# Kyaw-Thiha/animal-vision

Measured on AMD Instinct MI355X. Metric: megapixels/sec per-frame pipeline, higher is better.
Workload: dtype f16

## Files before the change

### animal-vision_amd/_lib.py

```python
from __future__ import annotations

import ctypes
import os

_HERE = os.path.dirname(os.path.abspath(__file__))
LIB_PATH = os.path.join(_HERE, "libavx.so")

AVX_OK = 0
AVX_ERR_INVALID, AVX_ERR_NO_DEVICE, AVX_ERR_HIP, AVX_ERR_UNSUPPORTED, AVX_ERR_NOMEM = -1, -2, -3, -4, -5
AVX_COLOR_MATRIX, AVX_COLOR_CAT_MERGE = 0, 1
AVX_POST_NONE, AVX_POST_GAUSS, AVX_POST_ROWGAIN, AVX_POST_STREAK = 0, 1, 2, 3
AVX_MAX_KSIZE = 33
AVX_PIX_FMTS = {"yuv420p": 0, "nv12": 1, "yuv422p": 2, "yuv444p": 3, "gray": 4, "yuv420p10le": 5, "yuv422p10le": 6, "yuv444p10le": 7,
                "p010le": 8}
AVX_TRANSFERS = {"pq": 1, "hlg": 2}
AVX_TONEMAPS = {"clip": 0, "mobius": 1}


class AvxError(RuntimeError):
    def __init__(self, code: int, msg: str):
        super().__init__(f"libavx error {code}: {msg}")
        self.code = code


# ... 339 lines not shown
    "avx_yuv_coefficients_d": (_i, [_i, _i, _i, ctypes.POINTER(ctypes.c_int), ctypes.POINTER(ctypes.c_int)]),
    "avx_yuv_frame_size": (_sz, [_i, _i, _i]),
    "avx_yuv_to_rgb_u8": (_i, [_vp, _i, _vp, _vp, _i, _i, _i, _i, _i, _vp]),
    "avx_rgb_to_yuv_u8": (_i, [_vp, _i, _vp, _vp, _i, _i, _i, _i, _i, _vp]),
    "avx_yuv_hdr_to_rgb_u8": (_i, [_vp, _i, _vp, _vp, _i, _i, _i, _i, _i, _i, ctypes.c_double, ctypes.c_double, _vp]),
    "avx_yuv_to_rgb_scaled_u8": (_i, [_vp, _i, _vp, _vp, _i, _i, _i, _i, _i, _i, _i, _vp]),
    "avx_yuv_hdr_to_rgb_scaled_u8": (_i, [_vp, _i, _vp, _vp, _i, _i, _i, _i, _i, _i, _i, _i, ctypes.c_double, ctypes.c_double, _vp]),
    "avx_frame_metrics_u8": (_i, [_vp, _vp, _vp, _i, _i, _i, _i, _vp, _vp]),
    "avx_plane_metrics": (_i, [_vp, _i, _vp, _i, _vp, _i, _i, _i, _i, _vp, _vp]),
    "avx_frame_metrics_ms_u8": (_i, [_vp, _vp, _vp, _i, _i, _i, _vp, _vp, _vp]),
    "avx_diff_map_u8": (_i, [_vp, _vp, _vp, _i, _i, _i, _i, ctypes.c_float, _i, _i, _vp, _vp, _vp, _vp]),
    "avx_delta_e_u8": (_i, [_vp, _vp, _vp, _i, _i, _i, _i, ctypes.c_float, ctypes.c_float, _i, _vp, _vp, _vp, _vp]),
    "avx_scielab_u8": (_i, [_vp, _vp, _vp, _i, _i, _i, ctypes.c_double, _i, ctypes.c_float, ctypes.c_float, _i, _vp, _vp, _vp, _vp]),
    "avx_remap_linear_planes": (_i, [_vp, _vp, _i, _i, _i, _vp, _vp, _vp, ctypes.c_float, _vp]),
    "avx_sobel3_plane": (_i, [_vp, _vp, _i, _i, _vp, _vp, _vp]),
    "avx_mst_gram": (_i, [_vp, _vp, _i, _sz, _i, _i, _vp, _vp, _vp, _vp]),
    "avx_mst_qkv_gram": (_i, [_vp, _vp, _vp, _sz, _i, _vp, _vp, _vp, _vp, _vp]),
    "avx_mst_qkv_gram16": (_i, [_vp, _vp, _vp, _sz, _i, _vp, _vp, _vp, _vp, _vp]),
    "avx_mst_ln_gemm_gelu": (_i, [_vp, _vp, _vp, _vp, ctypes.c_float, _vp, _sz, _i, _vp, _vp]),
    "avx_mst_convt2x2": (_i, [_vp, _vp, _vp, _vp, _vp, _i, _i, _i, _i, _vp]),
    "avx_mst_convt2x2_fuse": (_i, [_vp, _vp, _vp, _vp, _vp, _vp, _vp, _i, _i, _i, _i, _vp]),
    "avx_mst_posemb": (_i, [_vp, _vp, _vp, _vp, _vp, _vp, _vp, _i, _i, _i, _i, _vp]),
    "avx_mst_conv3x3_add": (_i, [_vp, _vp, _vp, _vp, _vp, _i, _i, _i, _i, _vp]),
    "avx_mst_attn_pack": (_i, [_vp, _vp, _vp, _vp, _vp, _vp, _i, _vp, _vp]),
    "avx_mst_rowgemm_add": (_i, [_vp, _vp, _vp, _vp, _vp, _vp, _vp, _sz, _i, _vp]),
    "avx_mst_conv_in_u8": (_i, [_vp, _vp, _i, _i, _i, _i, _i, _i, _vp, _vp, _vp]),
    "avx_mst_conv3x3_lds": (_i, [_vp, _vp, _vp, _vp, _vp, _i, _i, _i, _i, _vp]),
    "avx_mst_down4x4": (_i, [_vp, _vp, _vp, _vp, _i, _i, _i, _i, _vp]),
    "avx_mst_conv3x3_lds_gram": (_i, [_vp, _vp, _vp, _vp, _vp, _i, _i, _i, _vp, _vp, _vp, _vp, _vp]),
    "avx_mst_conv3x3_lds_cin": (_i, [_vp, _vp, _vp, _vp, _i, _i, _i, _i, _i, _i, _vp, _vp, _vp]),
    "avx_mst_conv3x3_lds_spectral_cin": (_i, [_vp, _vp, _vp, _vp, _i, _i, _i, _i, _i, _i, _vp, _fp, _i, _i, _i, _i, _vp, _vp, ctypes.POINTER(ctypes.c_int), _vp]),
    "avx_mst_conv3x3_lds_gram_cin": (_i, [_vp, _vp, _i, _i, _i, _i, _i, _i, _vp, _vp, _vp, _vp, _vp, _vp, _vp, _vp]),
    "avx_mst_convt2x2_fuse_gram": (_i, [_vp, _vp, _vp, _vp, _vp, _vp, _vp, _i, _i, _i, _vp, _vp, _vp, _vp, _vp]),
    "avx_mst_attn_pack16": (_i, [_vp, _vp, _vp, _vp, _vp, _vp, _i, _vp, _vp]),
    "avx_mst_attn_pack_mx": (_i, [_vp, _vp, _vp, _vp, _vp, _vp, _i, _vp, _vp]),
    "avx_mst_attn_tail_mx": (_i, [_vp, _vp, _vp, _vp, _vp, _vp, _vp, _vp, _i, _i, _i, _i, _vp]),
    "avx_mst_attn_tail_sp": (_i, [_vp, _vp, _vp, _vp, _vp, _vp, _vp, _vp, _i, _i, _i, _i, _vp]),
    "avx_mst_attn_tail_mx_col": (_i, [_vp, _vp, _vp, _vp, _vp, _vp, _vp, _vp, _i, _i, _i, _i, _i, _vp]),
    "avx_mst_attn_tail_sp_col": (_i, [_vp, _vp, _vp, _vp, _vp, _vp, _vp, _vp, _i, _i, _i, _i, _i, _vp]),
    "avx_mst_tail_march_steps": (_i, [_i, _i, _i, _i, ctypes.POINTER(ctypes.c_longlong), ctypes.POINTER(ctypes.c_ubyte), _i, ctypes.POINTER(ctypes.c_int)]),
    "avx_mst_attn_tail": (_i, [_vp, _vp, _vp, _vp, _vp, _vp, _vp, _vp, _i, _i, _i, _i, _vp]),
    "avx_mst_attn_tail_x": (_i, [_vp, _vp, _vp, _vp, _vp, _vp, _vp, _vp, _i, _i, _i, _i, _vp]),
    "avx_mst_ffn_fused": (_i, [_vp, _vp, _vp, _vp, ctypes.c_float, _vp, _vp, _vp, _vp, _i, _i, _i, _i, _vp]),
    "avx_mst_conv3x3_lds_spectral": (_i, [_vp, _vp, _vp, _vp, _i, _i, _i, _fp, _i, _i, _i, _i, _vp, _vp, ctypes.POINTER(ctypes.c_int), _vp]),
    "avx_mst_ffn_fused_mx": (_i, [_vp, _vp, _vp, _vp, ctypes.c_float, _vp, _vp, _vp, _vp, _i, _i, _i, _i, _vp]),
    "avx_mst_ffn_fused_sp": (_i, [_vp, _vp, _vp, _vp, ctypes.c_float, _vp, _vp, _vp, _vp, _i, _i, _i, _i, _vp]),
    "avx_mst_ffn_fused_mx_col": (_i, [_vp, _vp, _vp, _vp, ctypes.c_float, _vp, _vp, _vp, _vp, _i, _i, _i, _i, _i, _vp]),
    "avx_mst_ffn_fused_sp_col": (_i, [_vp, _vp, _vp, _vp, ctypes.c_float, _vp, _vp, _vp, _vp, _i, _i, _i, _i, _i, _vp]),
    "avx_mst_gelu_prescale": (ctypes.c_float, []),
    "avx_mst_tile_order": (_i, [_i, _i, _i, _i, _i, ctypes.POINTER(ctypes.c_longlong), _i, ctypes.POINTER(ctypes.c_int)]),
    "avx_mst_tile_order_col": (_i, [_i, _i, _i, _i, ctypes.POINTER(ctypes.c_longlong), ctypes.POINTER(ctypes.c_ubyte), _i, ctypes.POINTER(ctypes.c_int)]),
    "avx_mst_dw_gemm_add": (_i, [_vp, _vp, _vp, _vp, _vp, _vp, _i, _i, _i, _i, _vp]),
    "avx_dwconv3x3_nhwc_add": (_i, [_vp, _vp, _vp, _vp, _i, _i, _i, _i, _i, _vp, _vp, _vp]),
    "avx_dwconv3x3_nhwc": (_i, [_vp, _vp, _vp, _vp, _i, _i, _i, _i, _i, _i, _vp]),
    "avx_layernorm_rows": (_i, [_vp, _vp, _vp, _vp, _vp, _i, _sz, _i, ctypes.c_float, _vp]),
    "avx_layernorm_rows_grouped": (_i, [_vp, _vp, _vp, _vp, _vp, _i, _sz, _i, ctypes.c_float, _i, _i, _vp]),
}
for _name, (_res, _args) in _SIGS.items():
    _fn = getattr(lib, _name)
    _fn.restype = _res
    _fn.argtypes = _args

if lib.avx_abi_version() != 1:
    raise ImportError(f"libavx.so ABI {lib.avx_abi_version()} != 1 expected by this package: rebuild")
```

### animal-vision_amd/csrc/mst_mfma.hip

```cpp
#include <hip/hip_fp16.h>

#include "avx_internal.h"
#include "mst_common.h"

namespace {

constexpr int kT = 256;

__device__ __forceinline__ float16_t mfma(half4_t a, half4_t b, float16_t c) { return __builtin_amdgcn_mfma_f32_32x32x8f16(a, b, c, 0, 0, 0); }
__device__ __forceinline__ float16_t mfma16(half8_t a, half8_t b, float16_t c) { return __builtin_amdgcn_mfma_f32_32x32x16_f16(a, b, c, 0, 0, 0); }

template <int C>
__device__ __forceinline__ void load_x(const __half* __restrict__ x, size_t tile, size_t n, int lane, half4_t (&xf)[C / 8]) {
    const int p = lane & 31, h = lane >> 5;
    const size_t row = tile * 32 + p;
    if (row < n) {
        const uint4* src = reinterpret_cast<const uint4*>(x + row * (size_t)C + h * (C / 2));
#pragma unroll
        for (int q = 0; q < C / 16; ++q) {
            const uint4 v = src[q];
            const half8_t h8 = __builtin_bit_cast(half8_t, v);
            xf[2 * q] = half4_t{h8[0], h8[1], h8[2], h8[3]};
            xf[2 * q + 1] = half4_t{h8[4], h8[5], h8[6], h8[7]};
        }
// ... 699 lines not shown
                    dk = mfma16(o1, __builtin_bit_cast(half8_t, wq[3 * 64 + lane]), dk);
                    unsigned aq[8], ak[8];
#pragma unroll
                    for (int j = 0; j < 8; ++j) {
                        aq[j] = pack_f16(dq[2 * j], dq[2 * j + 1]);
                        ak[j] = pack_f16(dk[2 * j], dk[2 * j + 1]);
                        fma_mix_lo(nq, aq[j], aq[j]); fma_mix_hi(nq, aq[j], aq[j]);
                        fma_mix_lo(nk, ak[j], ak[j]); fma_mix_hi(nk, ak[j], ak[j]);
                    }
#pragma unroll
                    for (int b2 = 0; b2 < 2; ++b2)
                        G = mfma16(__builtin_bit_cast(half8_t, uint4{ak[4 * b2], ak[4 * b2 + 1], ak[4 * b2 + 2], ak[4 * b2 + 3]}),
                                   __builtin_bit_cast(half8_t, uint4{aq[4 * b2], aq[4 * b2 + 1], aq[4 * b2 + 2], aq[4 * b2 + 3]}), G);
                }
            }
        }
    }
    if constexpr (GRAM) {
        __syncthreads();
        float* red = reinterpret_cast<float*>(smem);
        float* mine = red + (size_t)wave * 34 * 32;
#pragma unroll
        for (int v = 0; v < 16; ++v) mine[(8 * (v / 4) + 4 * h + (v % 4)) * 32 + p] = G[v];
        const float sq = nq + __shfl_xor(nq, 32), sk = nk + __shfl_xor(nk, 32);
        if (h == 0) { mine[32 * 32 + p] = sq; mine[33 * 32 + p] = sk; }
        __syncthreads();
        for (int i = tid; i < 34 * 32; i += kT) {
            float sum = 0.f;
#pragma unroll
            for (int w4 = 0; w4 < 4; ++w4) sum += red[(size_t)w4 * 34 * 32 + i];
            partial[(size_t)blockIdx.x * 34 * 32 + i] = sum;
        }
    }
}

template <int C, int NW>
__global__ __launch_bounds__(64 * NW) void k_mst_qkv16(const __half* __restrict__ x, const uint4* __restrict__ wpack , size_t n,
                                                      __half* __restrict__ v_out , float* __restrict__ partial ) {
    constexpr int KS = C / 16, HD = C / 32, NT = 3 * HD;
    extern __shared__ __align__(16) unsigned char smem[];
    uint4* wl = reinterpret_cast<uint4*>(smem);
    const int tid = threadIdx.x, lane = tid & 63, wave = tid >> 6;
    for (int i = tid; i < NT * KS * 64; i += 64 * NW) wl[i] = wpack[i];
    __syncthreads();
    auto W = [&](int t, int s) { return __builtin_bit_cast(half8_t, wl[(t * KS + s) * 64 + lane]); };
    float16_t G[HD];
    float nq[HD], nk[HD];
#pragma unroll
    for (int hd = 0; hd < HD; ++hd) {
#pragma unroll
        for (int v = 0; v < 16; ++v) G[hd][v] = 0.f;
        nq[hd] = 0.f;
        nk[hd] = 0.f;
    }
    const size_t ntiles = (n + 31) / 32;
    const int p = lane & 31, h = lane >> 5;
    auto load_row = [&](size_t tile, uint4 (&u)[KS]) {
        const size_t row = tile * 32 + p;
        const uint4* src = reinterpret_cast<const uint4*>(x + (row < n ? row : n - 1) * (size_t)C + h * (C / 2));
#pragma unroll
        for (int q = 0; q < KS; ++q) u[q] = src[q];
    };
    constexpr bool PF = C <= 64;
    uint4 xn[KS];
    size_t tile = (size_t)blockIdx.x * NW + wave;
    if (PF && tile < ntiles) load_row(tile, xn);
// ... 318 lines not shown
    AVX_HIP(ctx, hipFuncSetAttribute((const void*)k, hipFuncAttributeMaxDynamicSharedMemorySize, (int)lds));
    hipLaunchKernelGGL(k, dim3((unsigned)blocks), dim3(kT), lds, s, (const __half*)x, (const uint2*)wpack, bias, (const __half*)skip, (const uint2*)wskip, (__half*)out, 1, H, W,
                       (const uint4*)wqk16, partial);
    AVX_HIP(ctx, hipGetLastError());
    return avx_mst_qkv_final_launch(ctx, partial, (int)blocks, 1, gram, nq, nk, s);
}
static int convt2x2_impl(avx_ctx* ctx, const void* x, const void* wpack, const float* bias, const void* skip, const void* wskip, void* out, int B, int H, int W,
                         int C, void* stream) {
    if (!ctx) return AVX_ERR_INVALID;
    AVX_REQUIRE(ctx, x && wpack && bias && out && B > 0 && H > 0 && W > 0, "avx_mst_convt2x2: NULL pointer or empty tensor");
    AVX_REQUIRE(ctx, C == 64 || C == 128, "avx_mst_convt2x2: C=%d (64 or 128 input channels)", C);
    AVX_REQUIRE(ctx, ((((uintptr_t)x | (uintptr_t)wpack | (uintptr_t)out)) & 15u) == 0, "avx_mst_convt2x2: pointers must be 16-byte aligned");
    AVX_HIP(ctx, hipSetDevice(ctx->device));
    hipStream_t s = avx_pick_stream(ctx, stream);
    const long total = (long)B * H * ((W + 31) / 32);
    long blocks = (total + 3) / 4;
    const long cap = (long)ctx->num_cus * (C == 128 ? 2 : 8);
    if (blocks > cap) blocks = cap;
    if (C == 64) {
        const size_t lds = (size_t)4 * 1 * 8 * 64 * sizeof(uint2) + sizeof(float) * 32 + (size_t)1 * 4 * 64 * sizeof(uint2);
        AVX_HIP(ctx, hipFuncSetAttribute((const void*)k_mst_convt2x2<64, false>, hipFuncAttributeMaxDynamicSharedMemorySize, (int)lds));
        hipLaunchKernelGGL((k_mst_convt2x2<64, false>), dim3((unsigned)blocks), dim3(kT), lds, s, (const __half*)x, (const uint2*)wpack, bias, (const __half*)skip,
                           (const uint2*)wskip, (__half*)out, B, H, W);
    } else {
        const size_t lds = (size_t)4 * 2 * 16 * 64 * sizeof(uint2) + sizeof(float) * 64 + (size_t)2 * 8 * 64 * sizeof(uint2);
        AVX_HIP(ctx, hipFuncSetAttribute((const void*)k_mst_convt2x2<128, false>, hipFuncAttributeMaxDynamicSharedMemorySize, (int)lds));
        hipLaunchKernelGGL((k_mst_convt2x2<128, false>), dim3((unsigned)blocks), dim3(kT), lds, s, (const __half*)x, (const uint2*)wpack, bias, (const __half*)skip,
                           (const uint2*)wskip, (__half*)out, B, H, W);
    }
    AVX_HIP(ctx, hipGetLastError());
    return AVX_OK;
}

}
```

### animal-vision_amd/ml/mst_plus_plus.py

```python
from __future__ import annotations

from typing import Dict, List

import torch
import torch.nn.functional as F

DIM = 31
PAD = 32


def padded(n: int) -> int:
    assert n % DIM == 0
    return n // DIM * PAD


def pad_index(n: int, device=None) -> torch.Tensor:
    i = torch.arange(n, device=device)
    return (i // DIM) * PAD + i % DIM


def pad_channels(t: torch.Tensor, dims) -> torch.Tensor:
    for d in dims:
        n = t.shape[d]
        shape = list(t.shape)
# ... 125 lines not shown
    return torch.stack([pack_fragments16(w[:, :, t // 4, t % 4].t().contiguous()) for t in range(16)]).contiguous()


class _AvxOps:

    def __init__(self):
        import os

        self.enabled = os.environ.get("AVX_MST_TORCH_ONLY", "") == ""
        self._mfma = os.environ.get("AVX_MST_NO_MFMA", "") == ""
        self._ffn2 = os.environ.get("AVX_MST_NO_FFN2", "") == ""
        self._posemb = os.environ.get("AVX_MST_NO_POSEMB", "") == ""
        self._conv_lds = os.environ.get("AVX_MST_NO_CONV_LDS", "") == ""
        self._conv_in = os.environ.get("AVX_MST_NO_CONV_IN", "") == ""
        self._upfuse = os.environ.get("AVX_MST_NO_UPFUSE", "") == ""
        self._tail = os.environ.get("AVX_MST_NO_TAIL", "") == ""
        self._tailx = os.environ.get("AVX_MST_NO_TAILX", "") == ""
        self._down = os.environ.get("AVX_MST_NO_DOWN4X4", "") == ""
        self._qkv16 = os.environ.get("AVX_MST_NO_QKV16", "") == ""
        self._convgram = os.environ.get("AVX_MST_NO_CONVGRAM", "") == ""
        self._ffn = os.environ.get("AVX_MST_NO_FFN_FUSED", "") == ""
        self._gelu_pre = None
        self._dwmx = os.environ.get("AVX_MST_NO_DW_MFMA", "") == ""
        self._dwsp = os.environ.get("AVX_MST_NO_DW_SPARSE", "") == ""
        self.DW_SPARSE_FFN_C = (32, 64, 128)
        self.DW_SPARSE_TAIL_C = (32, 64)
        self._specfuse = os.environ.get("AVX_MST_NO_SPEC_FUSE", "") == ""
        self._cinfuse = os.environ.get("AVX_MST_NO_CONV_IN_FUSE", "") == ""
        self.FFN_FUSED_C = tuple(int(v) for v in os.environ.get("AVX_MST_FFN_FUSED_C", "32,64,128").split(",") if v)
        self._ffn_march = os.environ.get("AVX_MST_NO_FFN_MARCH", "") == ""
        self.FFN_MARCH_C = (32, 64)
        self._tail_march = os.environ.get("AVX_MST_NO_TAIL_MARCH", "") == ""
        self.TAIL_MARCH_C = (32, 64)
        self._ctx = {}

    def ctx(self, device: torch.device):
        from ..runtime import get_context

        idx = device.index if device.index is not None else torch.cuda.current_device()
        c = get_context(idx)
        if c.device != idx:
            raise RuntimeError(f"libavx context is on device {c.device}, tensor on cuda:{idx} (one process per GPU)")
        return c

    @staticmethod
    def _dt(t: torch.Tensor) -> int:
        if t.dtype == torch.float32:
            return 0
        if t.dtype == torch.float16:
            return 1
        raise TypeError(f"csrc/mst.hip kernels take float32/float16, got {t.dtype}")

    def gram(self, qkv: torch.Tensor, heads: int):
        from .._lib import lib

        b, n, c3 = qkv.shape
        c = c3 // 3
        d = c // heads
        ctx = self.ctx(qkv.device)
        g = torch.empty((b, heads, 32, 32), dtype=torch.float32, device=qkv.device)
        nq = torch.empty((b, c), dtype=torch.float32, device=qkv.device)
        nk = torch.empty((b, c), dtype=torch.float32, device=qkv.device)
        st = torch.cuda.current_stream(qkv.device).cuda_stream
        for i in range(b):
            ctx._check(lib.avx_mst_gram(ctx._h, qkv[i].data_ptr(), self._dt(qkv), n, c, heads, g[i].data_ptr(), nq[i].data_ptr(), nk[i].data_ptr(), st))
        return g[:, :, :d, :d], nq, nk
# ... 34 lines not shown
                                            torch.cuda.current_stream(x2.device).cuda_stream))
        return out

    def convt2x2(self, x: torch.Tensor, wpack: torch.Tensor, bias: torch.Tensor, skip: torch.Tensor = None, wskip: torch.Tensor = None) -> torch.Tensor:
        from .._lib import lib

        b, h, w, c = x.shape
        x = x.contiguous()
        out = torch.empty((b, 2 * h, 2 * w, c // 2), dtype=torch.float16, device=x.device)
        ctx = self.ctx(x.device)
        st = torch.cuda.current_stream(x.device).cuda_stream
        if skip is None:
            ctx._check(lib.avx_mst_convt2x2(ctx._h, x.data_ptr(), wpack.data_ptr(), bias.data_ptr(), out.data_ptr(), b, h, w, c, st))
        else:
            assert skip.is_contiguous() and skip.shape == out.shape
            ctx._check(lib.avx_mst_convt2x2_fuse(ctx._h, x.data_ptr(), wpack.data_ptr(), bias.data_ptr(), skip.data_ptr(), wskip.data_ptr(), out.data_ptr(), b, h, w, c, st))
        return out

    def convt2x2_gram(self, x: torch.Tensor, wpack: torch.Tensor, bias: torch.Tensor, skip: torch.Tensor, wskip: torch.Tensor, wqk16: torch.Tensor):
        from .._lib import lib

        b, h, w, c = x.shape
        assert c == 64 and skip.is_contiguous() and skip.shape == (b, 2 * h, 2 * w, 32)
        x = x.contiguous()
        out = torch.empty((b, 2 * h, 2 * w, 32), dtype=torch.float16, device=x.device)
        g = torch.empty((b, 1, 32, 32), dtype=torch.float32, device=x.device)
        nq = torch.empty((b, 32), dtype=torch.float32, device=x.device)
        nk = torch.empty((b, 32), dtype=torch.float32, device=x.device)
        ctx = self.ctx(x.device)
        st = torch.cuda.current_stream(x.device).cuda_stream
        for i in range(b):
            ctx._check(lib.avx_mst_convt2x2_fuse_gram(ctx._h, x[i].data_ptr(), wpack.data_ptr(), bias.data_ptr(), skip[i].data_ptr(), wskip.data_ptr(), out[i].data_ptr(), h, w, c,
                                                      wqk16.data_ptr(), g[i].data_ptr(), nq[i].data_ptr(), nk[i].data_ptr(), st))
        return out, g, nq, nk

    def posemb(self, v: torch.Tensor, w1_c9: torch.Tensor, w2_c9: torch.Tensor, residual: torch.Tensor = None, bias: torch.Tensor = None) -> torch.Tensor:
        from .._lib import lib

        b, h, w, c = v.shape
        v = v.contiguous()
        residual = residual.contiguous() if residual is not None else None
        out = torch.empty_like(v)
        ctx = self.ctx(v.device)
        ctx._check(lib.avx_mst_posemb(ctx._h, v.data_ptr(), w1_c9.data_ptr(), w2_c9.data_ptr(), residual.data_ptr() if residual is not None else None,
                                      bias.data_ptr() if bias is not None else None, out.data_ptr(), b, h, w, c, torch.cuda.current_stream(v.device).cuda_stream))
        return out

    def conv3x3(self, x: torch.Tensor, wpack: torch.Tensor, add: torch.Tensor = None) -> torch.Tensor:
        from .._lib import lib

        b, h, w, c = x.shape
        x = x.contiguous()
        add = add.contiguous() if add is not None else None
        out = torch.empty_like(x)
        ctx = self.ctx(x.device)
        ctx._check(lib.avx_mst_conv3x3_add(ctx._h, x.data_ptr(), wpack.data_ptr(), add.data_ptr() if add is not None else None, out.data_ptr(), b, h, w, c,
                                           torch.cuda.current_stream(x.device).cuda_stream))
        return out

    def conv_in_u8(self, frame: torch.Tensor, pads, w_27x32: torch.Tensor) -> torch.Tensor:
        from .._lib import lib

        H, W, _ = frame.shape
        t, b, l, r = pads
        frame = frame.contiguous()
        out = torch.empty((1, H + t + b, W + l + r, 32), dtype=torch.float16, device=frame.device)
# ... 527 lines not shown
        x = self._ms_msa(x, p + ".blocks.0.0", heads, pre)
        return self._ffn(x, p + ".blocks.0.1")

    def _mst(self, x: torch.Tensor, p: str, src=None) -> torch.Tensor:
        pre = None
        ekey, a0 = p + ".embedding.weight", f"{p}.encoder_layers.0.0.blocks.0.0"
        if src is not None or (_AVX.fused_ok(x) and x.shape[-1] == 32 and _AVX._conv_lds and _AVX._convgram and _AVX._qkv16 and _AVX._tail and _AVX._tailx):
            wq = self._prep(ekey + ".frag9k16", lambda: torch.stack([pack_fragments16(self._w(ekey, (0, 1))[:, :, t // 3, t % 3].t().contiguous()) for t in range(9)]).contiguous())
            wqkv = self._prep(a0 + ".qkv", lambda: torch.cat([self._w(a0 + ".to_q.weight", (0, 1)), self._w(a0 + ".to_k.weight", (0, 1)),
                                                              self._w(a0 + ".to_v.weight", (0, 1))], 0).t().contiguous())
            wqk = self._prep(a0 + ".qkv.frag16", lambda: pack_qkv16(wqkv))
            fea, g, nq, nk = _AVX.conv3x3_lds_gram(x, wq, None, wqk) if src is None else _AVX.conv3x3_lds_gram_cin(src, wq, wqk)
            pre = (g, nq, nk)
        else:
            fea = self._conv3(x, ekey)
        skips: List[torch.Tensor] = []
        heads = 1
        for i in range(2):
            fea = self._msab(fea, f"{p}.encoder_layers.{i}.0", heads, pre if i == 0 else None)
            skips.append(fea)
            dkey = f"{p}.encoder_layers.{i}.1.weight"
            if _AVX.fused_ok(fea) and _AVX._down and fea.shape[-1] in (32, 64) and fea.is_contiguous():
                fea = _AVX.down4x4(fea, self._prep(dkey + ".frag16", lambda: pack_down4x4(self._w(dkey, (0, 1)))))
            else:
                fea = self._conv_nhwc(fea, self._w(dkey, (0, 1)), stride=2, padding=1)
            heads *= 2
        fea = self._msab(fea, p + ".bottleneck", heads)
        for i in range(2):
            kw = f"{p}.decoder_layers.{i}.0.weight"
            if _AVX.fused_ok(fea) and fea.shape[-1] in (64, 128) and _AVX._upfuse:
                ch = fea.shape[-1] // 2
                wfk = f"{p}.fuse{i}"
                wf_ = self._prep(wfk, lambda: self._w(f"{p}.decoder_layers.{i}.1.weight", (0, 1)).reshape(ch, 2 * ch).t().contiguous())
                gt = self._prep(kw + ".upfuse4", lambda: torch.stack([pack_fragments((self._w(kw, (0, 1))[:, :, t // 2, t % 2].float() @ wf_[:ch].float()).half().contiguous(), True)
                                                                     for t in range(4)]).contiguous())
                gb = self._prep(kw + ".upfuse.bias", lambda: (self._w(f"{p}.decoder_layers.{i}.0.bias", (0,)).float() @ wf_[:ch].float()).contiguous())
                wbot_ = self._prep(f"{p}.fuse{i}.bot", lambda: pack_fragments(wf_[ch:].contiguous(), True))
                heads //= 2
                a2 = f"{p}.decoder_layers.{i}.2.blocks.0.0"
                if ch == 32 and _AVX._convgram and _AVX._qkv16 and _AVX._tail and _AVX._tailx:
                    wqkv2 = self._prep(a2 + ".qkv", lambda: torch.cat([self._w(a2 + ".to_q.weight", (0, 1)), self._w(a2 + ".to_k.weight", (0, 1)),
                                                                       self._w(a2 + ".to_v.weight", (0, 1))], 0).t().contiguous())
                    wqk2 = self._prep(a2 + ".qkv.frag16", lambda: pack_qkv16(wqkv2))
                    fea, g2, nq2, nk2 = _AVX.convt2x2_gram(fea, gt, gb, skips[1 - i].contiguous(), wbot_, wqk2)
                    fea = self._msab(fea, f"{p}.decoder_layers.{i}.2", heads, (g2, nq2, nk2))
                    continue
                fea = _AVX.convt2x2(fea, gt, gb, skips[1 - i].contiguous(), wbot_)
                fea = self._msab(fea, f"{p}.decoder_layers.{i}.2", heads)
                continue
            if _AVX.fused_ok(fea) and fea.shape[-1] in (64, 128):
                wt = self._prep(kw + ".frag4", lambda: torch.stack([pack_fragments(self._w(kw, (0, 1))[:, :, t // 2, t % 2].contiguous(), True) for t in range(4)]).contiguous())
                bt = self._prep(kw + ".bias32", lambda: self._w(f"{p}.decoder_layers.{i}.0.bias", (0,)).float().contiguous())
                up = _AVX.convt2x2(fea, wt, bt)
            else:
                up = F.conv_transpose2d(fea.permute(0, 3, 1, 2), self._w(kw, (0, 1)), self._w(f"{p}.decoder_layers.{i}.0.bias", (0,)), stride=2).permute(0, 2, 3, 1)
            heads //= 2
            skip = skips[1 - i]
            b, h, w, ch = up.shape
            c2 = 2 * ch
            wf = self._prep(f"{p}.fuse{i}", lambda: self._w(f"{p}.decoder_layers.{i}.1.weight", (0, 1)).reshape(c2 // 2, c2).t().contiguous())
            if _AVX.fused_ok(skip):
                up, skip = up.contiguous(), skip.contiguous()
                wtop = self._prep(f"{p}.fuse{i}.top", lambda: pack_fragments(wf[:ch].contiguous(), True))
                wbot = self._prep(f"{p}.fuse{i}.bot", lambda: pack_fragments(wf[ch:].contiguous(), True))
                fea = _AVX.rowgemm_add(up.reshape(b * h * w, ch), wtop, None, skip.reshape(b * h * w, ch), wbot).reshape(b, h, w, ch)
            else:
                cat = torch.cat([up, skip], dim=-1)
                fea = (cat.reshape(b, h * w, c2) @ wf).reshape(b, h, w, c2 // 2)
            fea = self._msab(fea, f"{p}.decoder_layers.{i}.2", heads)
        if src is not None:
            return _AVX.conv3x3_lds_cin(fea, self._frag9k16(p + ".mapping.weight"), src)
        return self._conv3(fea, p + ".mapping.weight", add=x)

    @torch.no_grad()
    def forward_from_u8(self, frame: torch.Tensor, pads, spectral=None):
        w27 = self._prep("conv_in.w27x32", lambda: self._w("conv_in.weight", (0,)).permute(2, 3, 1, 0).reshape(27, PAD).float().contiguous())
        H, W, _ = frame.shape
        assert (H + pads[0] + pads[1]) % 8 == 0 and (W + pads[2] + pads[3]) % 8 == 0, "pad the frame to a multiple of 8 (predict_torch.py pads to 16)"
        spec = None if spectral is None else (spectral, (pads[0], pads[2], H, W))
        if self.can_fuse_conv_in_consumers():
            return self._body(None, spectral=spec, src=(frame, tuple(pads), w27))
# ... 32 lines not shown
        x = x.to(self._p("conv_in.weight").dtype).contiguous(memory_format=torch.channels_last).permute(0, 2, 3, 1)
        x = self._conv_nhwc(x, self._w("conv_in.weight", (0,)), padding=1)
        return self._body(x)[:, :h_inp, :w_inp, :]

    @torch.no_grad()
    def forward(self, x: torch.Tensor) -> torch.Tensor:
        return self.forward_nhwc(x)[..., :DIM].permute(0, 3, 1, 2)


def hbm_bytes_per_px(stage: int = 3) -> float:

    def msab(c: int) -> float:
        t = 2.0 * c
        if _AVX._tail and _AVX._tailx and (c in (32, 64) or (c == 128 and _AVX._dwmx)):
            b = t
            b += 2 * t
            return b + ((2 * t) if (_AVX._ffn and c in _AVX.FFN_FUSED_C) else (t + 4 * t + ((4 * t + 2 * t) if _AVX._ffn2 else (4 * t + 4 * t + 4 * t + 2 * t))))
        b = 2 * t
        if _AVX._tail and c in (32, 64):
            b += 3 * t
        else:
            b += (3 * t if _AVX._posemb else 5 * t)
            b += 3 * t
        if _AVX._ffn and c in _AVX.FFN_FUSED_C:
            b += 2 * t
        else:
            b += t + 4 * t
            b += (4 * t + 2 * t) if (c in (32, 64) and _AVX._ffn2) else (4 * t + 4 * t + 4 * t + 2 * t)
        return b

    per_stage = 2 * msab(32) + 2 * msab(64) / 4 + msab(128) / 16
    if _AVX._convgram and _AVX._qkv16 and _AVX._tail and _AVX._tailx and _AVX._conv_lds and _AVX._upfuse:
        per_stage -= 2 * 64.0
    t32, t64, t128 = 64.0, 128.0 / 4, 256.0 / 16
    convs = (2 * t32) + (3 * t32)
    convs += (t32 + t64) + (t64 + t128)
    if _AVX._upfuse:
        convs += (t128 + t64 + t64) + (t64 + t32 + t32)
    else:
        convs += (t128 + t64) + (2 * t64 + t64)
        convs += (t64 + t32) + (2 * t32 + t32)
    head = ((3 + t32) if _AVX._conv_in else (3 + 12) + (12 + t32)) + ((2 * t32 + 12) if (_AVX._specfuse and _AVX._conv_lds and _AVX._conv_in) else 3 * t32)
    if stage >= 1 and _AVX._cinfuse and _AVX._conv_in and _AVX._conv_lds and _AVX._convgram and _AVX._qkv16 and _AVX._tail and _AVX._tailx:
        head += 3 * 3 - (4 * t32 + 3)
    return stage * (per_stage + convs) + head
```

### include/avx.h

```cpp
#ifndef AVX_H
#define AVX_H

#include <stddef.h>
#include <stdint.h>

#ifdef __cplusplus
extern "C" {
#endif

#define AVX_ABI_VERSION 1

typedef struct avx_ctx avx_ctx;

typedef enum avx_status {
    AVX_OK = 0,
    AVX_ERR_INVALID = -1,
    AVX_ERR_NO_DEVICE = -2,
    AVX_ERR_HIP = -3,
    AVX_ERR_UNSUPPORTED = -4,
    AVX_ERR_NOMEM = -5
} avx_status;

int avx_abi_version(void);
int avx_device_count(void);
// ... 403 lines not shown
                         const void* w2pack, void* out, int B, int H, int W, int C, void* stream);
int avx_mst_ffn_fused_sp(avx_ctx* ctx, const void* x, const float* gamma, const float* beta, float eps, const void* w1pack, const void* dwpack,
                         const void* w2pack, void* out, int B, int H, int W, int C, void* stream);
float avx_mst_gelu_prescale(void);

int avx_mst_tile_order(int frames, int ty, int tx, int nwg, int raster, long long* visit, int steps_cap, int* steps_out);

int avx_mst_ffn_fused_mx_col(avx_ctx* ctx, const void* x, const float* gamma, const float* beta, float eps, const void* w1pack, const void* dwpack,
                             const void* w2pack, void* out, int B, int H, int W, int C, int max_workgroups, void* stream);
int avx_mst_ffn_fused_sp_col(avx_ctx* ctx, const void* x, const float* gamma, const float* beta, float eps, const void* w1pack, const void* dwpack,
                             const void* w2pack, void* out, int B, int H, int W, int C, int max_workgroups, void* stream);
int avx_mst_tile_order_col(int frames, int ty, int tx, int nwg, long long* visit, unsigned char* seg, int steps_cap, int* steps_out);

int avx_mst_attn_tail_mx_col(avx_ctx* ctx, const void* x, const void* wvpack16, const void* mpack_mx, const void* dw1pack, const void* dw2pack,
                             const float* bias, void* out, int B, int H, int W, int C, int max_workgroups, void* stream);
int avx_mst_attn_tail_sp_col(avx_ctx* ctx, const void* x, const void* wvpack16, const void* mpack_mx, const void* dw1pack, const void* dw2pack,
                             const float* bias, void* out, int B, int H, int W, int C, int max_workgroups, void* stream);
int avx_mst_tail_march_steps(int frames, int ty, int tx, int nwg, long long* visit, unsigned char* prime, int steps_cap, int* steps_out);

int avx_mst_rowgemm_add(avx_ctx* ctx, const void* a, const void* wpack, const void* a2, const void* wpack2, const void* add, void* out, size_t rows,
                        int C, void* stream);

int avx_mst_attn_pack(avx_ctx* ctx, const float* gram, const float* nq, const float* nk, const float* rescale, const float* wproj_t, int C,
                      void* mpack, void* stream);

int avx_mst_conv3x3_add(avx_ctx* ctx, const void* x, const void* wpack, const void* add, void* out, int B, int H, int W, int C, void* stream);

int avx_mst_posemb(avx_ctx* ctx, const void* v, const float* w1_c9, const float* w2_c9, const void* residual, const float* bias, void* out, int B,
                   int H, int W, int C, void* stream);

int avx_mst_convt2x2(avx_ctx* ctx, const void* x, const void* wpack, const float* bias, void* out, int B, int H, int W, int C, void* stream);
int avx_mst_convt2x2_fuse(avx_ctx* ctx, const void* x, const void* wpack, const float* bias, const void* skip, const void* wskip, void* out, int B, int H,
                          int W, int C, void* stream);

int avx_dwconv3x3_nhwc(avx_ctx* ctx, const void* x, const float* w_c9, void* y, int dtype, int B, int H, int W, int C, int gelu_out, void* stream);
int avx_dwconv3x3_nhwc_add(avx_ctx* ctx, const void* x, const float* w_c9, void* y, int B, int H, int W, int C, int gelu_out,
                           const void* residual, const float* bias, void* stream);

int avx_layernorm_rows(avx_ctx* ctx, const void* x, const float* gamma, const float* beta, void* y, int dtype, size_t rows, int C, float eps, void* stream);
int avx_layernorm_rows_grouped(avx_ctx* ctx, const void* x, const float* gamma, const float* beta, void* y, int dtype, size_t rows, int C, float eps,
                               int group, int real, void* stream);

int avx_get_table(int which, void* dst_host, size_t capacity);

#ifdef __cplusplus
}
#endif
#endif
```

Baseline: 453.6.

## Add K16 MFMA transposed-conv upsample kernel with fused skip and Gram epilogue

Result: faster. 458.8, median of 6 (+1.2%).

```diff
diff --git a/animal-vision_amd/_lib.py b/animal-vision_amd/_lib.py
--- a/animal-vision_amd/_lib.py
+++ b/animal-vision_amd/_lib.py
@@ -395,6 +395,8 @@
     "avx_mst_conv3x3_lds_spectral_cin": (_i, [_vp, _vp, _vp, _vp, _i, _i, _i, _i, _i, _i, _vp, _fp, _i, _i, _i, _i, _vp, _vp, ctypes.POINTER(ctypes.c_int), _vp]),
     "avx_mst_conv3x3_lds_gram_cin": (_i, [_vp, _vp, _i, _i, _i, _i, _i, _i, _vp, _vp, _vp, _vp, _vp, _vp, _vp, _vp]),
     "avx_mst_convt2x2_fuse_gram": (_i, [_vp, _vp, _vp, _vp, _vp, _vp, _vp, _i, _i, _i, _vp, _vp, _vp, _vp, _vp]),
+    "avx_mst_convt2x2_fuse16": (_i, [_vp, _vp, _vp, _vp, _vp, _vp, _vp, _i, _i, _i, _i, _vp]),
+    "avx_mst_convt2x2_fuse16_gram": (_i, [_vp, _vp, _vp, _vp, _vp, _vp, _vp, _i, _i, _i, _i, _vp, _vp, _vp, _vp, _vp]),
     "avx_mst_attn_pack16": (_i, [_vp, _vp, _vp, _vp, _vp, _vp, _i, _vp, _vp]),
     "avx_mst_attn_pack_mx": (_i, [_vp, _vp, _vp, _vp, _vp, _vp, _i, _vp, _vp]),
     "avx_mst_attn_tail_mx": (_i, [_vp, _vp, _vp, _vp, _vp, _vp, _vp, _vp, _i, _i, _i, _i, _vp]),
diff --git a/animal-vision_amd/csrc/mst_mfma.hip b/animal-vision_amd/csrc/mst_mfma.hip
--- a/animal-vision_amd/csrc/mst_mfma.hip
+++ b/animal-vision_amd/csrc/mst_mfma.hip
@@ -755,6 +755,180 @@
             partial[(size_t)blockIdx.x * 34 * 32 + i] = sum;
         }
     }
+}
+
+template <int C, int NW, bool SKIP, bool GRAM>
+__global__ __launch_bounds__(64 * NW, C == 64 ? 4 : 1) void k_mst_convt2x2_16(const __half* __restrict__ x , const uint4* __restrict__ wpack ,
+                                                            const float* __restrict__ bias , const __half* __restrict__ skip ,
+                                                            const uint4* __restrict__ wskip , __half* __restrict__ out , int B,
+                                                            int H, int W, const uint4* __restrict__ wqk , float* __restrict__ partial ) {
+    constexpr int KS = C / 16, CO = C / 2, NT = CO / 32, KSS = CO / 16, HD = NT;
+    static_assert(!GRAM || SKIP, "the Gram epilogue belongs to the fused decoder step");
+    extern __shared__ __align__(16) unsigned char smem[];
+    uint4* wl = reinterpret_cast<uint4*>(smem);
+    float* bl = reinterpret_cast<float*>(wl + 4 * NT * KS * 64);
+    uint4* wsl = reinterpret_cast<uint4*>(bl + CO);
+    uint4* wq = wsl + (SKIP ? NT * KSS * 64 : 0);
+    const int tid = threadIdx.x, lane = tid & 63, wave = tid >> 6;
+    for (int i = tid; i < 4 * NT * KS * 64; i += 64 * NW) wl[i] = wpack[i];
+    for (int i = tid; i < CO; i += 64 * NW) bl[i] = bias[i];
+    if constexpr (SKIP)
+        for (int i = tid; i < NT * KSS * 64; i += 64 * NW) wsl[i] = wskip[i];
+    float16_t G[GRAM ? HD : 1];
+    float nq[GRAM ? HD : 1], nk[GRAM ? HD : 1];
+    if constexpr (GRAM) {
+        for (int i = tid; i < 2 * HD * KSS * 64; i += 64 * NW) wq[i] = wqk[i];
+#pragma unroll
+        for (int hd = 0; hd < HD; ++hd) {
+#pragma unroll
+            for (int v = 0; v < 16; ++v) G[hd][v] = 0.f;
+            nq[hd] = 0.f;
+            nk[hd] = 0.f;
+        }
+    }
+    __syncthreads();
+    const int xt = (W + 31) / 32;
+    const long total = (long)B * H * xt;
+    const int p = lane & 31, h = lane >> 5;
+    for (long tile = (long)blockIdx.x * NW + wave; tile < total; tile += (long)gridDim.x * NW) {
+        const int x0 = (int)(tile % xt) * 32, y = (int)((tile / xt) % H);
+        const long b = tile / ((long)xt * H);
+        const int xw = x0 + p, xc = xw < W ? xw : W - 1;
+        uint4 xr[KS], sr[SKIP ? 4 : 1][KSS];
+        {
+            const uint4* src = reinterpret_cast<const uint4*>(x + (size_t)((b * H + y) * (long)W + xc) * C + h * (C / 2));
+#pragma unroll
+            for (int q = 0; q < KS; ++q) xr[q] = src[q];
+        }
+        const size_t opix0 = (size_t)(b * 2 * H + 2 * y) * (size_t)(2 * W) + (size_t)(2 * xc);
+        if constexpr (SKIP) {
+#pragma unroll
+            for (int tap = 0; tap < 4; ++tap) {
+                const uint4* src = reinterpret_cast<const uint4*>(skip + (opix0 + (size_t)(tap >> 1) * (size_t)(2 * W) + (tap & 1)) * CO + h * (CO / 2));
+#pragma unroll
+                for (int q = 0; q < KSS; ++q) sr[tap][q] = src[q];
+            }
+        }
+        asm volatile("" ::: "memory");
+#pragma unroll
+        for (int tap = 0; tap < 4; ++tap) {
+            const size_t opix = opix0 + (size_t)(tap >> 1) * (size_t)(2 * W) + (tap & 1);
+            uint4 og[NT][2];
+#pragma unroll
+            for (int t = 0; t < NT; ++t) {
+                float16_t d;
+#pragma unroll
+                for (int v = 0; v < 16; ++v) d[v] = 0.f;
+#pragma unroll
+                for (int s = 0; s < KS; ++s) d = mfma16(__builtin_bit_cast(half8_t, wl[((tap * NT + t) * KS + s) * 64 + lane]), __builtin_bit_cast(half8_t, xr[s]), d);
+                if constexpr (SKIP) {
+#pragma unroll
+                    for (int s = 0; s < KSS; ++s) d = mfma16(__builtin_bit_cast(half8_t, wsl[(t * KSS + s) * 64 + lane]), __builtin_bit_cast(half8_t, sr[tap][s]), d);
+                }
+                _Float16 o[16];
+#pragma unroll
+                for (int v = 0; v < 16; ++v) o[v] = (_Float16)(d[v] + bl[32 * t + 16 * h + v]);
+                if (xw < W) store_tile16(out + opix * CO + 32 * t + 16 * h, o);
+                if constexpr (GRAM) {
+                    half8_t o0, o1;
+#pragma unroll
+                    for (int v = 0; v < 8; ++v) { o0[v] = xw < W ? o[v] : (_Float16)0.f; o1[v] = xw < W ? o[8 + v] : (_Float16)0.f; }
+                    og[t][0] = __builtin_bit_cast(uint4, o0);
+                    og[t][1] = __builtin_bit_cast(uint4, o1);
+                }
+            }
+            if constexpr (GRAM) {
+                half8_t xq[KSS];
+                if constexpr (NT == 1) {
+                    xq[0] = __builtin_bit_cast(half8_t, og[0][0]);
+                    xq[1] = __builtin_bit_cast(half8_t, og[0][1]);
+                } else {
+                    unsigned a[8] = {og[0][0].x, og[0][0].y, og[0][0].z, og[0][0].w, og[0][1].x, og[0][1].y, og[0][1].z, og[0][1].w};
+                    unsigned c[8] = {og[1][0].x, og[1][0].y, og[1][0].z, og[1][0].w, og[1][1].x, og[1][1].y, og[1][1].z, og[1][1].w};
+#pragma unroll
+                    for (int i = 0; i < 8; ++i) {
+                        const auto r = __builtin_amdgcn_permlane32_swap(a[i], c[i], false, false);
+                        a[i] = r[0];
+                        c[i] = r[1];
+                    }
+                    xq[0] = __builtin_bit_cast(half8_t, uint4{a[0], a[1], a[2], a[3]});
+                    xq[1] = __builtin_bit_cast(half8_t, uint4{a[4], a[5], a[6], a[7]});
+                    xq[2] = __builtin_bit_cast(half8_t, uint4{c[0], c[1], c[2], c[3]});
+                    xq[3] = __builtin_bit_cast(half8_t, uint4{c[4], c[5], c[6], c[7]});
+                }
+#pragma unroll
+                for (int hd = 0; hd < HD; ++hd) {
+                    float16_t dq, dk;
+#pragma unroll
+                    for (int v = 0; v < 16; ++v) { dq[v] = 0.f; dk[v] = 0.f; }
+#pragma unroll
+                    for (int s = 0; s < KSS; ++s) dq = mfma16(xq[s], __builtin_bit_cast(half8_t, wq[(hd * KSS + s) * 64 + lane]), dq);
+#pragma unroll
+                    for (int s = 0; s < KSS; ++s) dk = mfma16(xq[s], __builtin_bit_cast(half8_t, wq[((HD + hd) * KSS + s) * 64 + lane]), dk);
+                    unsigned aq[8], ak[8];
+#pragma unroll
+                    for (int j = 0; j < 8; ++j) {
+                        aq[j] = pack_f16(dq[2 * j], dq[2 * j + 1]);
+                        ak[j] = pack_f16(dk[2 * j], dk[2 * j + 1]);
+                        fma_mix_lo(nq[hd], aq[j], aq[j]); fma_mix_hi(nq[hd], aq[j], aq[j]);
+                        fma_mix_lo(nk[hd], ak[j], ak[j]); fma_mix_hi(nk[hd], ak[j], ak[j]);
+                    }
+#pragma unroll
+                    for (int b2 = 0; b2 < 2; ++b2)
+                        G[hd] = mfma16(__builtin_bit_cast(half8_t, uint4{ak[4 * b2], ak[4 * b2 + 1], ak[4 * b2 + 2], ak[4 * b2 + 3]}),
+                                       __builtin_bit_cast(half8_t, uint4{aq[4 * b2], aq[4 * b2 + 1], aq[4 * b2 + 2], aq[4 * b2 + 3]}), G[hd]);
+                }
+            }
+        }
+    }
+    if constexpr (GRAM) {
+        __syncthreads();
+        float* red = reinterpret_cast<float*>(smem);
+#pragma unroll
+        for (int hd = 0; hd < HD; ++hd) {
+            float* mine = red + ((size_t)wave * HD + hd) * 34 * 32;
+#pragma unroll
+            for (int v = 0; v < 16; ++v) mine[(8 * (v / 4) + 4 * h + (v % 4)) * 32 + p] = G[hd][v];
+            const float sq = nq[hd] + __shfl_xor(nq[hd], 32), sk = nk[hd] + __shfl_xor(nk[hd], 32);
+            if (h == 0) { mine[32 * 32 + p] = sq; mine[33 * 32 + p] = sk; }
+        }
+        __syncthreads();
+        for (int i = tid; i < HD * 34 * 32; i += 64 * NW) {
+            float sum = 0.f;
+#pragma unroll
+            for (int w = 0; w < NW; ++w) sum += red[(size_t)w * HD * 34 * 32 + i];
+            partial[(size_t)blockIdx.x * HD * 34 * 32 + i] = sum;
+        }
+    }
+}
+
+template <int C, bool SKIP, bool GRAM> struct convt16_geom {
+    static constexpr int NW = C == 128 ? 8 : 4, PER_CU = C == 128 ? (SKIP ? 1 : 2) : 4;
+};
+
+template <int C, bool SKIP, bool GRAM>
+int launch_convt16(avx_ctx* ctx, avx_ws* ws, const void* x, const void* wpack, const float* bias, const void* skip, const void* wskip, void* out, int B, int H, int W,
+                   const void* wqk, float* gram, float* nq, float* nk, hipStream_t s) {
+    constexpr int NW = convt16_geom<C, SKIP, GRAM>::NW, KS = C / 16, CO = C / 2, NT = CO / 32, KSS = CO / 16, HD = NT;
+    size_t lds = sizeof(uint4) * ((size_t)4 * NT * KS * 64 + (SKIP ? NT * KSS * 64 : 0) + (GRAM ? 2 * HD * KSS * 64 : 0)) + sizeof(float) * CO;
+    if (GRAM && lds < sizeof(float) * NW * HD * 34 * 32) lds = sizeof(float) * NW * HD * 34 * 32;
+    const long total = (long)B * H * ((W + 31) / 32);
+    long blocks = (total + NW - 1) / NW;
+    const long cap = (long)ctx->num_cus * convt16_geom<C, SKIP, GRAM>::PER_CU;
+    if (blocks > cap) blocks = cap;
+    float* partial = nullptr;
+    if (GRAM) {
+        int rc = avx_ensure_scratch(ctx, ws, sizeof(float) * (size_t)blocks * HD * 34 * 32);
+        if (rc) return rc;
+        partial = (float*)ws->d_scratch;
+    }
+    auto k = k_mst_convt2x2_16<C, NW, SKIP, GRAM>;
+    AVX_HIP(ctx, hipFuncSetAttribute((const void*)k, hipFuncAttributeMaxDynamicSharedMemorySize, (int)lds));
+    hipLaunchKernelGGL(k, dim3((unsigned)blocks), dim3(64 * NW), lds, s, (const __half*)x, (const uint4*)wpack, bias, (const __half*)skip, (const uint4*)wskip, (__half*)out, B,
+                       H, W, (const uint4*)wqk, partial);
+    AVX_HIP(ctx, hipGetLastError());
+    if (GRAM) return avx_mst_qkv_final_launch(ctx, partial, (int)blocks, HD, gram, nq, nk, s);
+    return AVX_OK;
 }
 
 template <int C, int NW>
@@ -1139,4 +1313,36 @@
     return AVX_OK;
 }
 
-}
+int avx_mst_convt2x2_fuse16(avx_ctx* ctx, const void* x, const void* wpack16, const float* bias, const void* skip, const void* wskip16, void* out, int B, int H, int W,
+                            int C, void* stream) {
+    if (!ctx) return AVX_ERR_INVALID;
+    AVX_REQUIRE(ctx, x && wpack16 && bias && out && B > 0 && H > 0 && W > 0 && (!skip == !wskip16), "avx_mst_convt2x2_fuse16: NULL pointer or empty tensor");
+    AVX_REQUIRE(ctx, C == 64 || C == 128, "avx_mst_convt2x2_fuse16: C=%d (64 or 128 input channels)", C);
+    AVX_REQUIRE(ctx, ((((uintptr_t)x | (uintptr_t)wpack16 | (uintptr_t)out | (uintptr_t)skip | (uintptr_t)wskip16)) & 15u) == 0,
+                "avx_mst_convt2x2_fuse16: pointers must be 16-byte aligned");
+    AVX_HIP(ctx, hipSetDevice(ctx->device));
+    hipStream_t s = avx_pick_stream(ctx, stream);
+    if (C == 64) {
+        if (skip) return launch_convt16<64, true, false>(ctx, nullptr, x, wpack16, bias, skip, wskip16, out, B, H, W, nullptr, nullptr, nullptr, nullptr, s);
+        return launch_convt16<64, false, false>(ctx, nullptr, x, wpack16, bias, nullptr, nullptr, out, B, H, W, nullptr, nullptr, nullptr, nullptr, s);
+    }
+    if (skip) return launch_convt16<128, true, false>(ctx, nullptr, x, wpack16, bias, skip, wskip16, out, B, H, W, nullptr, nullptr, nullptr, nullptr, s);
+    return launch_convt16<128, false, false>(ctx, nullptr, x, wpack16, bias, nullptr, nullptr, out, B, H, W, nullptr, nullptr, nullptr, nullptr, s);
+}
+
+int avx_mst_convt2x2_fuse16_gram(avx_ctx* ctx, const void* x, const void* wpack16, const float* bias, const void* skip, const void* wskip16, void* out, int H, int W,
+                                 int C, int heads, const void* wqk16, float* gram, float* nq, float* nk, void* stream) {
+    if (!ctx) return AVX_ERR_INVALID;
+    AVX_REQUIRE(ctx, x && wpack16 && bias && skip && wskip16 && out && wqk16 && gram && nq && nk && H > 0 && W > 0, "avx_mst_convt2x2_fuse16_gram: NULL pointer or empty tensor");
+    AVX_REQUIRE(ctx, (C == 64 || C == 128) && heads == C / 64, "avx_mst_convt2x2_fuse16_gram: C=%d, heads=%d (64 or 128 input channels, one head per 32 output channels)", C, heads);
+    AVX_REQUIRE(ctx, ((((uintptr_t)x | (uintptr_t)wpack16 | (uintptr_t)out | (uintptr_t)skip | (uintptr_t)wskip16 | (uintptr_t)wqk16)) & 15u) == 0,
+                "avx_mst_convt2x2_fuse16_gram: pointers must be 16-byte aligned");
+    AVX_HIP(ctx, hipSetDevice(ctx->device));
+    hipStream_t s = avx_pick_stream(ctx, stream);
+    avx_ws* ws = avx_workspace(ctx, s);
+    if (!ws) return AVX_ERR_NOMEM;
+    if (C == 64) return launch_convt16<64, true, true>(ctx, ws, x, wpack16, bias, skip, wskip16, out, 1, H, W, wqk16, gram, nq, nk, s);
+    return launch_convt16<128, true, true>(ctx, ws, x, wpack16, bias, skip, wskip16, out, 1, H, W, wqk16, gram, nq, nk, s);
+}
+
+}
diff --git a/animal-vision_amd/ml/mst_plus_plus.py b/animal-vision_amd/ml/mst_plus_plus.py
--- a/animal-vision_amd/ml/mst_plus_plus.py
+++ b/animal-vision_amd/ml/mst_plus_plus.py
@@ -181,6 +181,9 @@
         self.FFN_MARCH_C = (32, 64)
         self._tail_march = os.environ.get("AVX_MST_NO_TAIL_MARCH", "") == ""
         self.TAIL_MARCH_C = (32, 64)
+        self._convt16 = os.environ.get("AVX_MST_NO_CONVT16", "") == ""
+        self.CONVT16_C = (64, 128)
+        self.CONVT16_GRAM_C = (128,)
         self._ctx = {}
 
     def ctx(self, device: torch.device):
@@ -281,6 +284,38 @@
         for i in range(b):
             ctx._check(lib.avx_mst_convt2x2_fuse_gram(ctx._h, x[i].data_ptr(), wpack.data_ptr(), bias.data_ptr(), skip[i].data_ptr(), wskip.data_ptr(), out[i].data_ptr(), h, w, c,
                                                       wqk16.data_ptr(), g[i].data_ptr(), nq[i].data_ptr(), nk[i].data_ptr(), st))
+        return out, g, nq, nk
+
+    def convt2x2_16(self, x: torch.Tensor, wpack16: torch.Tensor, bias: torch.Tensor, skip: torch.Tensor = None, wskip16: torch.Tensor = None) -> torch.Tensor:
+        from .._lib import lib
+
+        b, h, w, c = x.shape
+        x = x.contiguous()
+        out = torch.empty((b, 2 * h, 2 * w, c // 2), dtype=torch.float16, device=x.device)
+        ctx = self.ctx(x.device)
+        st = torch.cuda.current_stream(x.device).cuda_stream
+        if skip is not None:
+            assert skip.is_contiguous() and skip.shape == out.shape and wskip16 is not None
+        ctx._check(lib.avx_mst_convt2x2_fuse16(ctx._h, x.data_ptr(), wpack16.data_ptr(), bias.data_ptr(), skip.data_ptr() if skip is not None else None,
+                                               wskip16.data_ptr() if skip is not None else None, out.data_ptr(), b, h, w, c, st))
+        return out
+
+    def convt2x2_16_gram(self, x: torch.Tensor, wpack16: torch.Tensor, bias: torch.Tensor, skip: torch.Tensor, wskip16: torch.Tensor, wqk16: torch.Tensor):
+        from .._lib import lib
+
+        b, h, w, c = x.shape
+        ch, heads = c // 2, c // 64
+        assert c in (64, 128) and skip.is_contiguous() and skip.shape == (b, 2 * h, 2 * w, ch)
+        x = x.contiguous()
+        out = torch.empty((b, 2 * h, 2 * w, ch), dtype=torch.float16, device=x.device)
+        g = torch.empty((b, heads, 32, 32), dtype=torch.float32, device=x.device)
+        nq = torch.empty((b, ch), dtype=torch.float32, device=x.device)
+        nk = torch.empty((b, ch), dtype=torch.float32, device=x.device)
+        ctx = self.ctx(x.device)
+        st = torch.cuda.current_stream(x.device).cuda_stream
+        for i in range(b):
+            ctx._check(lib.avx_mst_convt2x2_fuse16_gram(ctx._h, x[i].data_ptr(), wpack16.data_ptr(), bias.data_ptr(), skip[i].data_ptr(), wskip16.data_ptr(), out[i].data_ptr(),
+                                                        h, w, c, heads, wqk16.data_ptr(), g[i].data_ptr(), nq[i].data_ptr(), nk[i].data_ptr(), st))
         return out, g, nq, nk
 
     def posemb(self, v: torch.Tensor, w1_c9: torch.Tensor, w2_c9: torch.Tensor, residual: torch.Tensor = None, bias: torch.Tensor = None) -> torch.Tensor:
@@ -874,21 +909,29 @@
                 ch = fea.shape[-1] // 2
                 wfk = f"{p}.fuse{i}"
                 wf_ = self._prep(wfk, lambda: self._w(f"{p}.decoder_layers.{i}.1.weight", (0, 1)).reshape(ch, 2 * ch).t().contiguous())
-                gt = self._prep(kw + ".upfuse4", lambda: torch.stack([pack_fragments((self._w(kw, (0, 1))[:, :, t // 2, t % 2].float() @ wf_[:ch].float()).half().contiguous(), True)
-                                                                     for t in range(4)]).contiguous())
                 gb = self._prep(kw + ".upfuse.bias", lambda: (self._w(f"{p}.decoder_layers.{i}.0.bias", (0,)).float() @ wf_[:ch].float()).contiguous())
-                wbot_ = self._prep(f"{p}.fuse{i}.bot", lambda: pack_fragments(wf_[ch:].contiguous(), True))
                 heads //= 2
                 a2 = f"{p}.decoder_layers.{i}.2.blocks.0.0"
-                if ch == 32 and _AVX._convgram and _AVX._qkv16 and _AVX._tail and _AVX._tailx:
+                cangram = _AVX._convgram and _AVX._qkv16 and _AVX._tail and _AVX._tailx
+                gram16 = cangram and _AVX._convt16 and 2 * ch in _AVX.CONVT16_C and 2 * ch in _AVX.CONVT16_GRAM_C
+                gram8 = cangram and ch == 32 and not gram16
+                k16 = gram16 or (_AVX._convt16 and 2 * ch in _AVX.CONVT16_C and not gram8)
+                tap = lambda t: (self._w(kw, (0, 1))[:, :, t // 2, t % 2].float() @ wf_[:ch].float()).half().contiguous()
+                if k16:
+                    gt = self._prep(kw + ".upfuse4k16", lambda: torch.stack([pack_fragments16(tap(t), halfrow=True) for t in range(4)]).contiguous())
+                    wbot_ = self._prep(f"{p}.fuse{i}.bot16", lambda: pack_fragments16(wf_[ch:].contiguous(), halfrow=True))
+                else:
+                    gt = self._prep(kw + ".upfuse4", lambda: torch.stack([pack_fragments(tap(t), True) for t in range(4)]).contiguous())
+                    wbot_ = self._prep(f"{p}.fuse{i}.bot", lambda: pack_fragments(wf_[ch:].contiguous(), True))
+                pre2 = None
+                if gram16 or gram8:
                     wqkv2 = self._prep(a2 + ".qkv", lambda: torch.cat([self._w(a2 + ".to_q.weight", (0, 1)), self._w(a2 + ".to_k.weight", (0, 1)),
                                                                        self._w(a2 + ".to_v.weight", (0, 1))], 0).t().contiguous())
                     wqk2 = self._prep(a2 + ".qkv.frag16", lambda: pack_qkv16(wqkv2))
-                    fea, g2, nq2, nk2 = _AVX.convt2x2_gram(fea, gt, gb, skips[1 - i].contiguous(), wbot_, wqk2)
-                    fea = self._msab(fea, f"{p}.decoder_layers.{i}.2", heads, (g2, nq2, nk2))
-                    continue
-                fea = _AVX.convt2x2(fea, gt, gb, skips[1 - i].contiguous(), wbot_)
-                fea = self._msab(fea, f"{p}.decoder_layers.{i}.2", heads)
+                    fea, *pre2 = (_AVX.convt2x2_16_gram if gram16 else _AVX.convt2x2_gram)(fea, gt, gb, skips[1 - i].contiguous(), wbot_, wqk2)
+                else:
+                    fea = (_AVX.convt2x2_16 if k16 else _AVX.convt2x2)(fea, gt, gb, skips[1 - i].contiguous(), wbot_)
+                fea = self._msab(fea, f"{p}.decoder_layers.{i}.2", heads, tuple(pre2) if pre2 else None)
                 continue
             if _AVX.fused_ok(fea) and fea.shape[-1] in (64, 128):
                 wt = self._prep(kw + ".frag4", lambda: torch.stack([pack_fragments(self._w(kw, (0, 1))[:, :, t // 2, t % 2].contiguous(), True) for t in range(4)]).contiguous())
@@ -987,6 +1030,8 @@
     per_stage = 2 * msab(32) + 2 * msab(64) / 4 + msab(128) / 16
     if _AVX._convgram and _AVX._qkv16 and _AVX._tail and _AVX._tailx and _AVX._conv_lds and _AVX._upfuse:
         per_stage -= 2 * 64.0
+        if _AVX._convt16 and 128 in _AVX.CONVT16_C and 128 in _AVX.CONVT16_GRAM_C:
+            per_stage -= 128.0 / 4
     t32, t64, t128 = 64.0, 128.0 / 4, 256.0 / 16
     convs = (2 * t32) + (3 * t32)
     convs += (t32 + t64) + (t64 + t128)
diff --git a/include/avx.h b/include/avx.h
--- a/include/avx.h
+++ b/include/avx.h
@@ -459,6 +459,10 @@
 int avx_mst_convt2x2(avx_ctx* ctx, const void* x, const void* wpack, const float* bias, void* out, int B, int H, int W, int C, void* stream);
 int avx_mst_convt2x2_fuse(avx_ctx* ctx, const void* x, const void* wpack, const float* bias, const void* skip, const void* wskip, void* out, int B, int H,
                           int W, int C, void* stream);
+int avx_mst_convt2x2_fuse16(avx_ctx* ctx, const void* x, const void* wpack16, const float* bias, const void* skip, const void* wskip16, void* out, int B, int H,
+                            int W, int C, void* stream);
+int avx_mst_convt2x2_fuse16_gram(avx_ctx* ctx, const void* x, const void* wpack16, const float* bias, const void* skip, const void* wskip16, void* out, int H, int W,
+                                 int C, int heads, const void* wqk16, float* gram, float* nq, float* nk, void* stream);
 
 int avx_dwconv3x3_nhwc(avx_ctx* ctx, const void* x, const float* w_c9, void* y, int dtype, int B, int H, int W, int C, int gelu_out, void* stream);
 int avx_dwconv3x3_nhwc_add(avx_ctx* ctx, const void* x, const float* w_c9, void* y, int B, int H, int W, int C, int gelu_out,
```
